# sashashura/h2o-3

Hardware: AMD Instinct MI355X
Metric: gbm_trees_per_sec (higher is better)
Workload: dtype fp32; 1 GPU; model=GBM binomial 100Mx100 ntrees=500 max_depth=8, rows=100000000, cols=100, max_depth=8, histogram_type=QuantilesGlobal, nbins=255, global_batch=100000000, parallelism=dp1

## Files before the change

h2o3_amd/models/tree/devtree.py:

```python
from __future__ import annotations

import os

import numpy as np
import torch

from ...ops import _native, tree_ops
from ...ops._native import check as _ck, ptr as _ptr, stream as _stream
from ...parallel import cloud
from ...parallel import collectives as coll
from ...utils import graphs
from .engine import _TreeBuf
from .record import FEAT, GAIN, OPT, T, rec_cols

RS = 16
_RC = rec_cols(2)
L0, L1, R0, R1, T0, T1, OK, NL, NAW = _RC.L, _RC.L + 1, _RC.R, _RC.R + 1, _RC.TOT, _RC.TOT + 1, _RC.OK, _RC.NL, _RC.NAW
ST, CT, VAL = range(_RC.width, RS)
MAX_DEPTH = 11


def _libs():
    return tree_ops._lib(), _native.get_lib("tree_split")

# ... 113 lines not shown
        self.fbase = torch.zeros(self.cap_p, dtype=i32, device=dev)
        self.lwork = torch.zeros(self.cap_l * 4, dtype=i32, device=dev)
        self.counts = torch.zeros(2, dtype=i32, device=dev)
        self.cnt = torch.zeros(self.cap_p, dtype=i32, device=dev)
        self.loff = torch.zeros(self.cap_p, dtype=i32, device=dev)
        self.roff = torch.zeros(self.cap_p, dtype=i32, device=dev)
        self.flags = torch.zeros(N // 64 + self.cap_p + 1, dtype=torch.int64, device=dev)
        self.part = self.plan_r.part(cap_h, dev)
        self.split_out = torch.zeros(n_lvl_max * max(self.Fl, 1) * 4, dtype=f64, device=dev)
        self.mask = torch.zeros(n_lvl_max * Bs, dtype=torch.uint8, device=dev)
        self.feat_i = torch.zeros(n_lvl_max, dtype=i32, device=dev)
        self.okm = torch.ones((n_lvl_max, max(self.Fl, 1)), dtype=torch.uint8, device=dev)
        if self.f0 + self.Fl > self.F:
            self.okm[:, max(0, self.F - self.f0):] = 0
        self._okm_col = None
        self.mono = torch.zeros(max(self.Fl, 1), dtype=torch.float32, device=dev)
        if bd.codes_col is not None:
            self.pcodes, self.prs, self.pfs = bd.codes_col, 1, bd.nrows_local
        else:
            self.pcodes, self.prs, self.pfs = bd.codes, bd.Fp, 1
        self.cutmat = g._cut_matrix()
        self.sampled = not drv._unit_weights
        self.wbuf = torch.ones(N, dtype=torch.float32, device=dev) if self.sampled else None
        self.colsamp = gp.col_sample_rate < 1.0 or gp.col_sample_rate_change_per_level != 1.0
        if self.colsamp:
            self.cs_elig = torch.zeros(max(self.F, 1), dtype=torch.int64, device=dev)
            self.cs_m = torch.zeros(1, dtype=torch.int32, device=dev)
            self.cs_k = torch.zeros(max(D, 1), dtype=torch.int32, device=dev)
            self.cs_seed = torch.zeros(max(D, 1), dtype=torch.int64, device=dev)
        self.gather = os.environ.get("H2O3_LEAF_GATHER", "1") != "0" and N > 0
        self.last_level = self.gather and os.environ.get("H2O3_DEV_LAST_LEVEL", "1") != "0"
        self.lg = LeafGather(self.lh, N, D, dev) if self.gather else None
        self.slot_wb = torch.zeros(n_lvl_max, dtype=i32, device=dev)
        self.graph = None
        self._hv = [None, None]
        self._k = 0

    def _scales(self):
        self.sc_r = self.plan_r.scales(self.vmax)
        self.sc_c = self.plan_c.scales(self.vmax)

    def set_tree_cols(self, mask):
        key = None if mask is None else mask.tobytes()
        if key == self._okm_col:
            return
        self._okm_col = key
        m = np.ones(self.Fpad, dtype=np.uint8)
        if mask is not None:
            m[:self.F] = np.asarray(mask, dtype=np.uint8)
        m[self.F:] = 0
        row = self._upload([m[self.f0:self.f0 + self.Fl].copy()])[0]
        self.okm.copy_(row.view(1, -1).expand_as(self.okm))

    def _upload(self, arrays):
        offs, n = [], 0
        for a in arrays:
            offs.append(n)
            n += (a.nbytes + 7) & ~7
        n = max(n, 8)
        if getattr(self, "_stg", None) is None or self._stg[0].numel() < n:
            self._stg = [torch.empty(n, dtype=torch.uint8, pin_memory=True) for _ in range(2)]
            self._stg_ev = [None, None]
            self._dstg = torch.empty(n, dtype=torch.uint8, device=self.dev)
            self._stg_i = 0
        i = self._stg_i
        self._stg_i ^= 1
# ... 68 lines not shown
        gains = g[:, :, :8].contiguous().view(torch.float64).view(W, n)
        best = torch.argmax(gains, 0)
        win = g[best, torch.arange(n, device=buf.device)]
        pk = win[:, :rb].contiguous().view(torch.float64).view(n, 13)
        rows[:, :13].copy_(pk)
        self.mask[:n * Bs].view(n, Bs).copy_(win[:, rb:])
        okf = pk[:, OK] > 0
        self.feat_i[:n].copy_(torch.where(okf, pk[:, FEAT], torch.zeros_like(pk[:, FEAT])).to(torch.int32))

    def _level(self, d, cur):
        lh, ls, gp = self.lh, self.ls, self.gp
        n = 1 << d
        Bs = self.Bs
        H, wyy = self._hist(d, cur)
        recl = self._rec_lvl(d)
        s = _stream()
        if self.colsamp:
            rp = self._rec_lvl(d - 1) if d > 0 else None
            _ck(lh.h2o_dt_colmask(d, _ptr(rp), _ptr(self.cs_elig), _ptr(self.cs_m), _ptr(self.cs_k),
                                  _ptr(self.cs_seed), self.f0, self.Fl, _ptr(self.okm), s), "dt_colmask")
        _ck(ls.h2o_split_find_b(_ptr(H), self.Fl, n, Bs, _ptr(wyy), _ptr(self.okm), _ptr(self.mono),
                                float(gp.min_rows), float(gp.min_split_improvement), float(gp.reg_lambda),
                                float(gp.reg_alpha), float(gp.gamma), 0, _ptr(self.split_out), None, 0, s),
            "split_find")
        _ck(ls.h2o_split_select2(_ptr(self.split_out), _ptr(H), self.Fl, n, Bs, self.f0, 2.0 * float(gp.min_rows), RS,
                                 _ptr(recl), _ptr(self.mask), _ptr(self.feat_i), s), "split_select2")
        if self.W > 1:
            self._merge(recl, n)
        s = _stream()
        skip = self.last_level and d == self.D - 1
        _ck(lh.h2o_dt_items2(0, _ptr(recl), n, self.D, 0, self.chunk_p, self.cap_p, _ptr(self.pwork),
                             _ptr(self.fbase), _ptr(self.slot_wb) if skip else None, _ptr(self.counts), s),
            "dt_items(part)")
        _ck(lh.h2o_part_flags(_ptr(self.pcodes), 1, self.prs, self.pfs, _ptr(self._ridx(d, cur)),
                              _ptr(self.pwork), _ptr(self.fbase), self.cap_p, _ptr(self.feat_i), _ptr(self.mask),
                              Bs, _ptr(self.flags), _ptr(self.cnt), _ptr(self.counts), s), "part_flags")
        _ck(lh.h2o_dt_offsets(_ptr(self.cnt), _ptr(self.pwork), _ptr(self.counts), _ptr(recl), n,
                              _ptr(self._rec_lvl(d + 1)), _ptr(self.loff), _ptr(self.roff), s), "dt_offsets")
        if skip:
            _ck(lh.h2o_leaf_flag_sums_dev(_ptr(self.pos[cur]), _ptr(self.pwork), _ptr(self.fbase), self.cap_p,
                                          _ptr(self.flags), _ptr(recl), self.D, 1 if self.bern else 0,
                                          _ptr(self.sums), _ptr(self.counts), s), "leaf_flag_sums_dev")
            return cur
        nxt = cur ^ 1
        if d == 0 and self.root_ident:
            _ck(lh.h2o_dt_root_leaf_iota(_ptr(recl), _ptr(self.ridx[0]), self.N, s), "dt_root_leaf_iota")
        _ck(lh.h2o_part_compact(_ptr(self._ridx(d, cur)), _ptr(self.pwork), _ptr(self.fbase), self.cap_p,
                                _ptr(self.flags), _ptr(self.loff), _ptr(self.roff), _ptr(self.ridx[nxt]),
                                _ptr(self.pos[cur]), _ptr(self.pos[nxt]), _ptr(self.counts), s),
            "part_compact")
        return nxt

    def _sequence(self):
        lh, drv = self.lh, self.drv
        s = _stream()
        y = drv.yb if self.bern else torch.nan_to_num(drv.yf)
        if not hasattr(self, "_y"):
            self._y = y.contiguous().to(torch.float32)
        f = drv._f[:, 0]
        _ck(lh.h2o_gbm_grad(_ptr(self._y), _ptr(f), _ptr(self.wbuf) if self.sampled else None,
                            1 if self.bern else 0, self.N, _ptr(self.pos[0]), _ptr(self.dbuf), s), "gbm_grad")
        if not self.root_ident:
            _ck(lh.h2o_iota_i32(_ptr(self.ridx[0]), self.N, s), "iota")
        self.rec.zero_()
        self.sums.zero_()
        _ck(lh.h2o_dt_root(_ptr(self.rec), self.N, _stream()), "dt_root")
        cur = 0
        for d in range(self.D):
            cur = self._level(d, cur)
# ... 126 lines not shown
```

h2o3_amd/ops/_abi.py:

```python
import ctypes

_TABLE = {
    "dl": """
        h2o_dl_seed_advance  i  PP
        h2o_dl_fwd           i  PPPiiifQPifP
        h2o_dl_bwd           i  PPPPPiiifQPP
        h2o_dl_update        i  PPPPPPPPPiifffffffiiiffP
        h2o_dl_softmax       i  PPPPPPPiifiP
        h2o_dl_mlp_step      i  iPPPPPPPPPPPPPPPiPPPPiifQPiP
        h2o_dl_gemm_ws       q  iii
        h2o_dl_gemm          i  iiiPqqPqqPPqP
    """,
    "dl_shap": """
        h2o_dl_shap_chunk  i
        h2o_dl_shap_lds    q  iP
        h2o_dl_shap_pairs  i  iPPPPPPPPPPiiPPqqqiiP
    """,
    "fairness": """
        h2o_fairness_lds_groups  i
        h2o_group_sketch         i  PiPPqiiidiPPPiP
    """,
    "frame": """
        h2o_rollup_multi    i  PiqiPiPP
        h2o_expand_numeric  i  PiqPPPPiiiP
# ... 6 lines not shown
        h2o_glm_wide_split_grid  i  i
        h2o_glm_wide_split       i  PiiiqPfPPPiiffPPiPPP
        h2o_glm_wide_gram        i  PiiqPiiPiP
        h2o_glm_wide_gram256     i  PiiqPiiPiiP
        h2o_gram_f64             i  PiiqPPiiqPP
        h2o_xv_f64               i  PiiqPdPP
        h2o_xtr_f64              i  PiiqPiqPP
    """,
    "kmeans": """
        h2o_kmeans_assign_resident_per_cu  i  ii
        h2o_kmeans_assign                  i  PqiPPiPPiP
        h2o_xv_resident_per_cu             i  ii
        h2o_xv                             i  PqiPiPiP
        h2o_kmeans_max_k                   i  ii
        h2o_kmeans_part_stride             q  ii
        h2o_kmeans_set_debug               v  i
        h2o_kmeans_resident_per_cu         i  iiif
        h2o_kmeans_lloyd                   i  PPqiPPiPPPPiifP
        h2o_kmeans_sums_resident_per_cu    i  ii
        h2o_kmeans_sums                    i  PPqiiPPPPifP
        h2o_kmeans_reduce                  i  PiqPP
    """,
    "metrics": """
        h2o_logit_hist    i  PPPqiPPP
        h2o_group_reduce  i  PPqiiiPP
    """,
    "tree_hist": """
        h2o_hist_quad           i  PiPPPPiiiiffPiiiPiqiiPPP
        h2o_hist_bm_set_debug   v  i
        h2o_hist_bm             i  PiPPPPiiiiffPiiPiqiiiPPPP
        h2o_iota_i32            i  PqP
        h2o_hist_build          i  PiiPPPPiiiiffPiiiPiPP
        h2o_hist_build_pk       i  PiiPPPPiiiifqPiiPiPP
        h2o_part_flags          i  PiqqPPPiPPiPPPP
        h2o_hist_sibling        i  PPPiiiiiiiPPPPPP
        h2o_child_work          i  PPPiiiiiiiiPPPP
        h2o_part_offsets        i  PPiiPPPPiiP
        h2o_part_compact        i  PPPiPPPPPPPP
        h2o_part_count          i  PiqqPPiPPiPP
        h2o_part_scatter        i  PiqqPPiPPiPPPPPPPP
        h2o_fill_nid            i  PPiPP
        h2o_leaf_pass           i  PPPPiiPPP
        h2o_seg_sum2            i  PPPPiPP
        h2o_leaf_pos            i  PPiiPPP
        h2o_col_sample          i  iiPiQPP
        h2o_leaf_scatter        i  PPiPPP
        h2o_leaf_update         i  PPiPPP
        h2o_pair_hist4          i  PiqPPPPiPiiiffPPPP
        h2o_pair_hist           i  PiqPPPPiPiiiffPPP
        h2o_gbm_grad            i  PPPiqPPP
        h2o_part_items          i  PiiiPPPP
        h2o_dt_items2           i  iPiiiiiPPPPP
        h2o_dt_items            i  iPiiiiiPPPP
        h2o_dt_offsets          i  PPPPiPPPP
        h2o_dt_sibling          i  PPPiiiiiiPPPPP
        h2o_dt_leaf_vals        i  PPiiPdPP
        h2o_dt_root             i  PqP
        h2o_dt_root_leaf_iota   i  PPqP
        h2o_leaf_scatter_dev    i  PPiPPPP
        h2o_leaf_flag_sums_dev  i  PPPiPPiiPPP
        h2o_leaf_gather_lds     i  ii
        h2o_leaf_gather_items   i  qi
        h2o_leaf_gather_dev     i  PiiiPPPPqiiPPPPPP
        h2o_dt_colmask          i  iPPPPPiiPP
    """,
    "tree_pd": """
        h2o_pd_block_threads  i  ii
# ... 48 lines not shown
```

h2o3_amd/ops/csrc/tree_hist.hip:

```cpp
#include "common.h"
#include <stdlib.h>
#include <algorithm>

template <int MODE> struct Chan { static constexpr int C = MODE == 2 ? 1 : 2; };

template <typename CodeT, int MODE, bool HAS_VB, bool POSV, bool PACK = false>
__global__ __launch_bounds__(512) void hist_build_kernel(
    const CodeT* __restrict__ codes, int Fp, const int* __restrict__ ridx,
    const float* __restrict__ va, const float* __restrict__ vb,
    const int4* __restrict__ work, int F, int Bs, int FGL, float s0, float s1,
    double* __restrict__ hist, int n_slots, double* __restrict__ wyy_out, const uint8_t* __restrict__ need,
    long long bq = 0) {
  constexpr int C = Chan<MODE>::C;
  constexpr int CL = PACK ? 1 : C;
  const int RPW = 64 / FGL;
  extern __shared__ __attribute__((aligned(16))) unsigned long long ldsq[];
  const int4 wk = work[blockIdx.x];
  if (need != nullptr && need[(size_t)wk.x * gridDim.y + blockIdx.y] == 0) return;
  const int fg0 = blockIdx.y * FGL;
  const int nf = min(FGL, F - fg0);
  const int stride_f = Bs * CL;
  const int total = FGL * stride_f;
  for (int i = threadIdx.x; i < total; i += blockDim.x) ldsq[i] = 0ull;
  __syncthreads();
// ... 823 lines not shown
    int wpre = 0, tot = 0;
#pragma unroll
    for (int w = 0; w < 4; ++w) {
      const int s = wsum[w];
      wpre += (w < wv) ? s : 0;
      tot += s;
    }
    const int lpre = wpre + incl - nl;
    const int tile_first = base;
    const int pos_before = max(0, min(p0, end) - tile_first);
    int li = lbase + lpre;
    int ri = rbase + (pos_before - lpre);
    if (p0 < end) {
#pragma unroll
      for (int k = 0; k < 16; ++k) {
        if (p0 + k < end) {
          const int dst = ((bits >> k) & 1u) ? li++ : ri++;
          out[dst] = r[k];
          if (pa) { pa_out[dst] = pa[p0 + k]; pb_out[dst] = pb[p0 + k]; }
        }
      }
    }
    const int tile_n = min(256 * 16, end - base);
    lbase += tot;
    rbase += tile_n - tot;
    __syncthreads();
  }
}
template <typename CodeT>
__global__ __launch_bounds__(256) void part_flags_kernel(
    const CodeT* __restrict__ codes, long long rs, long long fs, const int* __restrict__ ridx,
    const int4* __restrict__ work, const int* __restrict__ fbase, const int* __restrict__ feat,
    const uint8_t* __restrict__ masks, int Bs, unsigned long long* __restrict__ flags, int* __restrict__ cnt,
    const int* __restrict__ nw_dev) {
  __shared__ uint8_t m[4096];
  __shared__ int red[4];
  if (nw_dev != nullptr && (int)blockIdx.x >= nw_dev[1]) return;
  const int4 wk = work[blockIdx.x];
  const int f = feat[wk.x];
  for (int i = threadIdx.x; i < Bs; i += blockDim.x) m[i] = masks[(size_t)wk.x * Bs + i];
  __syncthreads();
  const int lane = threadIdx.x & 63, wv = threadIdx.x >> 6;
  const int end = wk.y + wk.z;
  const int fb = fbase[blockIdx.x];
  int local = 0;
  constexpr int U = 8;
  for (int base = wk.y; base < end; base += 256 * U) {
    int r[U], c[U];
#pragma unroll
    for (int u = 0; u < U; ++u) {
      const int pc = min(base + u * 256 + (int)threadIdx.x, end - 1);
      r[u] = ridx != nullptr ? ridx[pc] : pc;
    }
#pragma unroll
    for (int u = 0; u < U; ++u) c[u] = (int)codes[(size_t)r[u] * rs + (size_t)f * fs];
#pragma unroll
    for (int u = 0; u < U; ++u) {
      const int p = base + u * 256 + (int)threadIdx.x;
      const bool L = p < end && m[c[u]];
      const unsigned long long bal = __ballot(L);
      const int w0 = base + u * 256 + wv * 64;
      if (lane == 0 && w0 < end) flags[fb + (w0 - wk.y) / 64] = bal;
      local += L ? 1 : 0;
    }
  }
  local = (int)wave_sum((float)local);
  if (lane == 0) red[wv] = local;
  __syncthreads();
  if (threadIdx.x == 0) cnt[blockIdx.x] = red[0] + red[1] + red[2] + red[3];
}
// ... 235 lines not shown
}

extern "C" {

int h2o_iota_i32(int* out, long long n, hipStream_t s) {
  if (n <= 0) return 0;
  if (((uintptr_t)out & 15) != 0) return -1;
  const long long blocks = std::min<long long>((n / 4 + 255) / 256 + 1, 4096);
  hipLaunchKernelGGL(iota_i32_kernel, dim3((unsigned)blocks), dim3(256), 0, s, out, n);
  return (int)hipGetLastError();
}

int h2o_hist_build(const void* codes, int code_bytes, int Fp, const int* ridx, const float* va,
                   const float* vb, const int* work, int n_work, int F, int FG, int Bs, float s0, float s1,
                   double* hist, int n_slots, int mode, int threads, double* wyy, int posv, const uint8_t* need,
                   hipStream_t s) {
  if (n_work <= 0) return 0;
  if (code_bytes == 1)
    return launch_hist<uint8_t>(codes, Fp, ridx, va, vb, (const int4*)work, n_work, F, FG, Bs, s0, s1, hist, n_slots, mode, threads, wyy, posv, need, s);
  return launch_hist<uint16_t>(codes, Fp, ridx, va, vb, (const int4*)work, n_work, F, FG, Bs, s0, s1, hist, n_slots, mode, threads, wyy, posv, need, s);
}

int h2o_hist_build_pk(const void* codes, int code_bytes, int Fp, const int* ridx, const float* va,
                      const float* vb, const int* work, int n_work, int F, int FG, int Bs, float s1, long long bq,
                      double* hist, int n_slots, int threads, double* wyy, int posv, const uint8_t* need,
                      hipStream_t s) {
  if (n_work <= 0) return 0;
  if (bq < 0) return (int)hipErrorInvalidValue;
  if (code_bytes == 1)
    return launch_hist<uint8_t>(codes, Fp, ridx, va, vb, (const int4*)work, n_work, F, FG, Bs, 1.f, s1, hist, n_slots,
                                0, threads, wyy, posv, need, s, bq);
  return launch_hist<uint16_t>(codes, Fp, ridx, va, vb, (const int4*)work, n_work, F, FG, Bs, 1.f, s1, hist, n_slots,
                               0, threads, wyy, posv, need, s, bq);
}

int h2o_part_flags(const void* codes, int code_bytes, long long rs, long long fs, const int* ridx,
                   const int* work, const int* fbase, int n_work, const int* feat, const uint8_t* masks, int Bs,
                   unsigned long long* flags, int* cnt, const int* counts, hipStream_t s) {
  if (n_work <= 0) return 0;
  if (code_bytes == 1)
    hipLaunchKernelGGL(part_flags_kernel<uint8_t>, dim3(n_work), dim3(256), 0, s, (const uint8_t*)codes, rs, fs,
                       ridx, (const int4*)work, fbase, feat, masks, Bs, flags, cnt, counts);
  else
    hipLaunchKernelGGL(part_flags_kernel<uint16_t>, dim3(n_work), dim3(256), 0, s, (const uint16_t*)codes, rs, fs,
                       ridx, (const int4*)work, fbase, feat, masks, Bs, flags, cnt, counts);
  return (int)hipGetLastError();
}

int h2o_hist_sibling(const double* Hb, const double* Hp, const int* slots, int nb, int np, int nf, int F, int BsC,
                     int C, int clamp_mask, double* H, const double* wyy_b, const double* wyy_p, double* wyy_out,
                     const int* counts, hipStream_t s) {
  if (nb <= 0 || F <= 0) return 0;
  hipLaunchKernelGGL(hist_sibling_kernel, dim3(nb, F), dim3(256), 0, s, Hb, Hp, slots, nb, np, nf, BsC, C, clamp_mask,
                     H, wyy_b, wyy_p, wyy_out, counts);
  return (int)hipGetLastError();
}

__global__ __launch_bounds__(1024) void child_work_kernel(const long long* __restrict__ st,
                                                          const long long* __restrict__ ct,
                                                          const double* __restrict__ rec, int stride, int ok_col,
                                                          int nl_col, int wl_col, int wr_col, int n, int chunk,
                                                          int cap, int4* __restrict__ work, int* __restrict__ slots,
                                                          int* __restrict__ counts) {
  __shared__ long long wtot[2][16];
  __shared__ long long carry[2];
  const int lane = threadIdx.x & 63, wv = threadIdx.x >> 6, nwv = blockDim.x >> 6;
  if (threadIdx.x == 0) carry[0] = carry[1] = 0;
  __syncthreads();
  for (int base = 0; base < n; base += blockDim.x) {
    const int i = base + threadIdx.x;
    long long sp = 0, nch = 0, start = 0, cnt = 0;
    bool bl = true;
    if (i < n && rec[(size_t)i * stride + ok_col] > 0) {
      const long long nl = (long long)rec[(size_t)i * stride + nl_col];
      bl = rec[(size_t)i * stride + wl_col] <= rec[(size_t)i * stride + wr_col];
      cnt = bl ? nl : ct[i] - nl;
      start = bl ? st[i] : st[i] + nl;
      sp = 1;
      nch = (cnt + chunk - 1) / chunk;
// ... 926 lines not shown
      }
      sl[u] = a;
      p[u] = lo[a] + (j - pre[a]);
    }
#pragma unroll
    for (int u = 0; u < U; ++u) r[u] = ridx[p[u]];
#pragma unroll
    for (int u = 0; u < U; ++u) {
      const int4 sg = segs[sl[u]];
      int h = sg.x;
      if (sg.w >= 0) {
        const int q = p[u] - sg.y;
        h = 2 * h + (((flags[sg.w + (q >> 6)] >> (q & 63)) & 1ull) ? 1 : 2);
      }
      const long long li = (long long)r[u] - row0;
      if (j0 + u * nt < total && li >= 0 && li < nrows) v[li] = __float_as_uint(vals[h]);
    }
  }
  __syncthreads();
  float* dr = d + row0;
  for (int i = threadIdx.x * 4; i < nrows; i += nt * 4) {
    const uint4 q = *reinterpret_cast<const uint4*>(v + i);
    if (i + 3 < nrows && q.x != LG_NONE && q.y != LG_NONE && q.z != LG_NONE && q.w != LG_NONE) {
      *reinterpret_cast<uint4*>(dr + i) = q;
    } else {
      const unsigned int e[4] = {q.x, q.y, q.z, q.w};
#pragma unroll
      for (int k = 0; k < 4; ++k)
        if (i + k < nrows && e[k] != LG_NONE) dr[i + k] = __uint_as_float(e[k]);
    }
  }
}

extern "C" {

int h2o_dt_items2(int kind, const double* rec, int n, int D, int wch, int chunk, int cap, int* work, int* fbase,
                  int* slot_wb, int* counts, hipStream_t s) {
  if (n <= 0 || n > DT_MAXN || chunk <= 0 || (fbase != nullptr && chunk % 64 != 0)) return -1;
  hipLaunchKernelGGL(dt_items_kernel, dim3(1), dim3(1024), 0, s, kind, rec, n, D, wch, chunk, cap, (int4*)work, fbase,
                     slot_wb, counts);
  return (int)hipGetLastError();
}

int h2o_dt_items(int kind, const double* rec, int n, int D, int wch, int chunk, int cap, int* work, int* fbase,
                 int* counts, hipStream_t s) {
  return h2o_dt_items2(kind, rec, n, D, wch, chunk, cap, work, fbase, nullptr, counts, s);
}

int h2o_dt_offsets(const int* cnt, const int* work, const int* counts, double* rec, int n, double* rec_next, int* loff,
                   int* roff, hipStream_t s) {
  if (n <= 0 || n > DT_MAXN) return -1;
  hipLaunchKernelGGL(dt_offsets_kernel, dim3(1), dim3(1024), 0, s, cnt, (const int4*)work, counts, rec, n, rec_next,
                     loff, roff);
  return (int)hipGetLastError();
}

int h2o_dt_sibling(const double* Hb, const double* Hp, const double* rec_par, int np, int F, int BsC, int C,
                   int clamp_mask, int wch, double* H, const double* wyy_b, const double* wyy_p, double* wyy_out,
                   hipStream_t s) {
  if (np <= 0 || F <= 0) return 0;
  hipLaunchKernelGGL(dt_sibling_kernel, dim3(np, F), dim3(256), 0, s, Hb, Hp, rec_par, np, BsC, C, clamp_mask, wch, H,
                     wyy_b, wyy_p, wyy_out);
  return (int)hipGetLastError();
}

int h2o_dt_leaf_vals(double* rec, const double* sums, int nh, int D, const float* lr, double maxabs, float* vals,
                     hipStream_t s) {
// ... 135 lines not shown
```

h2o3_amd/ops/tree_ops.py:

```python
from __future__ import annotations

import math
import os
from typing import NamedTuple

import numpy as np
import torch

from . import _native
from ._native import check as _check, ptr as _ptr, stream as _stream

_LDS_BUDGET = 80 * 1024


_upload_seq = 0
_synced_upto = 0


def upload_mark():
    return _upload_seq


def host_synced(mark=None):
    global _synced_upto
# ... 517 lines not shown
    lib = _lib()
    yc, fc = y.contiguous().to(torch.float32), f.contiguous().to(torch.float32)
    wc = w.contiguous().to(torch.float32) if w is not None else None
    _check(lib.h2o_gbm_grad(_ptr(yc), _ptr(fc), _ptr(wc), mode, n, _ptr(z), _ptr(d), _stream()), "h2o_gbm_grad")
    return z


def partition(bd, ridx, ridx_out, feats, masks, starts, counts, use_native=None, chunk=16384, payload=None):
    dev = ridx.device
    n = len(starts)
    if n == 0:
        return []
    native = dev.type == "cuda" if use_native is None else use_native
    if native:
        lib = _lib()
        items = make_work(starts, counts, range(n), chunk)
        if len(items) == 0:
            return [0] * n
        work = _h2d(items, dev)
        nw = len(items)
        feat_t = _h2d(np.asarray(feats, dtype=np.int32), dev)
        masks = masks.to(torch.uint8).contiguous()
        cnt = torch.empty(nw, dtype=torch.int32, device=dev)
        if bd.codes_col is not None:
            codes, rs, fs = bd.codes_col, 1, bd.nrows_local
        else:
            codes, rs, fs = bd.codes, bd.Fp, 1
        ballot = env("H2O3_PART", "ballot") == "ballot" and (payload is None or payload[1] is None)
        if ballot:
            words = (items[:, 2].astype(np.int64) + 63) // 64
            fb_h = (np.cumsum(words) - words).astype(np.int32)
            fbase = _h2d(fb_h, dev)
            flags = torch.empty(int(words.sum()) + 1, dtype=torch.int64, device=dev)
            rc = lib.h2o_part_flags(_ptr(codes), bd.code_bytes, rs, fs, _ptr(ridx), _ptr(work), _ptr(fbase), nw,
                                    _ptr(feat_t), _ptr(masks), bd.Bs, _ptr(flags), _ptr(cnt), None, _stream())
        else:
            rc = lib.h2o_part_count(_ptr(codes), bd.code_bytes, rs, fs, _ptr(ridx), _ptr(work), nw, _ptr(feat_t),
                                    _ptr(masks), bd.Bs, _ptr(cnt), _stream())
        _check(rc, "h2o_part_count")
        cnt_h = cnt.cpu().numpy().astype(np.int64)
        slot = items[:, 0].astype(np.int64)
        nleft = np.bincount(slot, weights=cnt_h, minlength=n).astype(np.int64)
        csum = np.cumsum(cnt_h) - cnt_h
        first = np.ones(len(items), dtype=bool)
        first[1:] = slot[1:] != slot[:-1]
        first_idx = np.maximum.accumulate(np.where(first, np.arange(len(items)), 0))
        lpre = csum - csum[first_idx]
        st_arr = np.asarray(starts, dtype=np.int64)[slot]
        rpre = (items[:, 1].astype(np.int64) - st_arr) - lpre
        loff = (st_arr + lpre).astype(np.int32)
        roff = (st_arr + nleft[slot] + rpre).astype(np.int32)
        loff_d = _h2d(loff, dev)
        roff_d = _h2d(roff, dev)
        pa, pb, pa_o, pb_o = payload if payload is not None else (None, None, None, None)
        if ballot:
            _check(lib.h2o_part_compact(_ptr(ridx), _ptr(work), _ptr(fbase), nw, _ptr(flags), _ptr(loff_d),
                                        _ptr(roff_d), _ptr(ridx_out), _ptr(pa), _ptr(pa_o), None, _stream()),
                   "h2o_part_compact")
            return nleft.tolist()
        _check(lib.h2o_part_scatter(_ptr(codes), bd.code_bytes, rs, fs, _ptr(ridx), _ptr(work), nw, _ptr(feat_t),
                                    _ptr(masks), bd.Bs, _ptr(loff_d), _ptr(roff_d), _ptr(ridx_out), _ptr(pa), _ptr(pb),
                                    _ptr(pa_o), _ptr(pb_o), _stream()), "h2o_part_scatter")
        return nleft.tolist()
    out = []
    for i, (st, ct) in enumerate(zip(starts, counts)):
        seg = ridx[st: st + ct]
        if bd.codes_col is not None:
            c = bd.codes_col[feats[i]][seg.long()].to(torch.int64)
        else:
            c = bd.codes[seg.long(), feats[i]].to(torch.int64)
        left = masks[i].to(torch.bool)[c]
        l = seg[left]
        r = seg[~left]
        ridx_out[st: st + l.numel()] = l
        ridx_out[st + l.numel(): st + ct] = r
        if payload is not None:
            pa, pb, pa_o, pb_o = payload
            for src, dst in ((pa, pa_o), (pb, pb_o)):
                v = src[st: st + ct]
                dst[st: st + l.numel()] = v[left]
                dst[st + l.numel(): st + ct] = v[~left]
        out.append(int(l.numel()))
    return out


def _part_chunk(total):
    ev = env("H2O3_PART_CHUNK")
    if ev:
        return int(ev)
    return int(max(4096, min(16384, -(-int(total) // 2048 // 64) * 64)))


def iota_i32(out) -> bool:
    lib = _lib()
    if lib is None or out.dtype != torch.int32 or not out.is_cuda or out.data_ptr() % 16:
        return False
    return lib.h2o_iota_i32(_ptr(out), out.numel(), _stream()) == 0


def partition_async(bd, ridx, ridx_out, feat_d, masks, starts, counts, chunk=None, payload=None, pk=None,
                    pk_col=0):
    dev = ridx.device
    n = len(starts)
    lib = _lib()
    if chunk is None:
        chunk = _part_chunk(sum(counts))
    nleft = torch.empty(n, dtype=torch.int64, device=dev)
    st = np.asarray(starts, dtype=np.int64).reshape(-1)
    ct = np.asarray(counts, dtype=np.int64).reshape(-1)
    nch = (ct + chunk - 1) // chunk
    nw = int(nch.sum())
    if nw == 0:
        nleft.zero_()
        if pk is not None:
            pk[:, pk_col] = 0.0
        return nleft
    wd = (ct + 63) // 64
    total_words = int(wd.sum())
    buf = torch.empty(13 * nw, dtype=torch.int32, device=dev)
    meta = buf[: 8 * nw].view(torch.int64)
    work = buf[8 * nw: 12 * nw]
    fbase = buf[12 * nw:]
    if chunk % 64 == 0 and env("H2O3_PART_ITEMS", "dev") == "dev":
        seg = _h2d(np.concatenate([st, ct, np.cumsum(nch) - nch, np.cumsum(wd) - wd]), dev)
        _check(lib.h2o_part_items(_ptr(seg), n, chunk, nw, _ptr(work), _ptr(meta), _ptr(fbase), _stream()),
               "h2o_part_items")
    else:
        items = make_work(starts, counts, range(n), chunk)
        words = (items[:, 2].astype(np.int64) + 63) // 64
        fb_h = (np.cumsum(words) - words).astype(np.int64)
        slot = items[:, 0].astype(np.int64)
        first = np.ones(nw, dtype=bool)
        first[1:] = slot[1:] != slot[:-1]
        first_idx = np.maximum.accumulate(np.where(first, np.arange(nw), 0))
        st_arr = st[slot]
        pos = items[:, 1].astype(np.int64) - st_arr
        buf.copy_(_h2d(np.concatenate([np.stack([slot, first_idx, st_arr, pos], 0).reshape(-1).view(np.int32),
                                       items.reshape(-1), fb_h.astype(np.int32)]), dev))
    feat_t = feat_d if feat_d.dtype == torch.int32 else feat_d.to(torch.int32)
    masks = masks if masks.dtype == torch.uint8 else masks.to(torch.uint8)
    cnt = torch.empty(nw, dtype=torch.int32, device=dev)
    if bd.codes_col is not None:
        codes, rs, fs = bd.codes_col, 1, bd.nrows_local
    else:
        codes, rs, fs = bd.codes, bd.Fp, 1
    flags = torch.empty(total_words + 1, dtype=torch.int64, device=dev)
    _check(lib.h2o_part_flags(_ptr(codes), bd.code_bytes, rs, fs, _ptr(ridx), _ptr(work), _ptr(fbase), nw,
                              _ptr(feat_t), _ptr(masks), bd.Bs, _ptr(flags), _ptr(cnt), None, _stream()),
           "h2o_part_flags")
    loff = torch.empty(nw, dtype=torch.int32, device=dev)
    roff = torch.empty(nw, dtype=torch.int32, device=dev)
    stride = pk.stride(0) if pk is not None else 0
    _check(lib.h2o_part_offsets(_ptr(cnt), _ptr(meta), nw, n, _ptr(loff), _ptr(roff), _ptr(nleft), _ptr(pk),
                                stride, pk_col, _stream()), "h2o_part_offsets")
    pa, _, pa_o, _ = payload if payload is not None else (None, None, None, None)
    _check(lib.h2o_part_compact(_ptr(ridx), _ptr(work), _ptr(fbase), nw, _ptr(flags), _ptr(loff), _ptr(roff),
                                _ptr(ridx_out), _ptr(pa), _ptr(pa_o), None, _stream()), "h2o_part_compact")
    return nleft


def hist_build_dev(bd, ridx, va, vb, mode, rec, rec_cols, starts, counts, vmax, posv=False, unit_w=False,
                   target_blocks=None):
    dev = ridx.device
    if dev.type != "cuda":
        return None
    total = int(sum(counts))
    plan = hist_plan(bd, mode, unit_w, (total + 1) // 2, target_blocks)
    if plan.kernel not in ("bm", "quad"):
        return None
    lib = _lib()
    n = len(starts)
    C = channels(mode)
    chunk = plan.chunk
    cap = n + total // chunk + 1
    stc = np.concatenate([np.asarray(starts, dtype=np.int64), np.asarray(counts, dtype=np.int64)])
    stc_d = _h2d(stc, dev)
    ibuf = torch.empty(4 * cap + 3 * n + 2, dtype=torch.int32, device=dev)
    work, slots, cnts = ibuf[:4 * cap], ibuf[4 * cap:4 * cap + 3 * n], ibuf[4 * cap + 3 * n:]
    ok_c, nl_c, wl_c, wr_c = rec_cols
    _check(lib.h2o_child_work(_ptr(stc_d), _ptr(stc_d[n:]), _ptr(rec), rec.stride(0), ok_c, nl_c, wl_c, wr_c, n, chunk,
                              cap, _ptr(work), _ptr(slots), _ptr(cnts), _stream()), "h2o_child_work")
# ... 166 lines not shown
```

Before: 69.94 trees/s.

## Add slab-based partition flag kernel that streams feature columns through LDS windows

Adds a row-slab partition-flags path for deep levels (depth >= 5, up to 1024 nodes) with column-major 1-byte codes. Each block loads a 64K-row window of one split feature's codes into LDS and classifies the rows that fall in that window. This replaces scattered random gathers from huge feature columns with coalesced streaming reads. A device-side rule decides whether to use the slab path, based on distinct features versus rows, and falls back to the original kernel otherwise. The cost is extra small kernels (rule, zero, binary-search bounds), atomics on flags and counts, and high LDS use.

```diff
diff --git a/h2o3_amd/models/tree/devtree.py b/h2o3_amd/models/tree/devtree.py
--- a/h2o3_amd/models/tree/devtree.py
+++ b/h2o3_amd/models/tree/devtree.py
@@ -169,6 +169,7 @@
         self.last_level = self.gather and os.environ.get("H2O3_DEV_LAST_LEVEL", "1") != "0"
         self.lg = LeafGather(self.lh, N, D, dev) if self.gather else None
         self.slot_wb = torch.zeros(n_lvl_max, dtype=i32, device=dev)
+        self.slab = tree_ops.PartSlab(N, n_lvl_max, dev) if bd.codes_col is not None and N > 0 else None
         self.graph = None
         self._hv = [None, None]
         self._k = 0
@@ -303,9 +304,10 @@
         _ck(lh.h2o_dt_items2(0, _ptr(recl), n, self.D, 0, self.chunk_p, self.cap_p, _ptr(self.pwork),
                              _ptr(self.fbase), _ptr(self.slot_wb) if skip else None, _ptr(self.counts), s),
             "dt_items(part)")
-        _ck(lh.h2o_part_flags(_ptr(self.pcodes), 1, self.prs, self.pfs, _ptr(self._ridx(d, cur)),
-                              _ptr(self.pwork), _ptr(self.fbase), self.cap_p, _ptr(self.feat_i), _ptr(self.mask),
-                              Bs, _ptr(self.flags), _ptr(self.cnt), _ptr(self.counts), s), "part_flags")
+        slab = self.slab if self.slab is not None and self.slab.eligible(d) else None
+        _ck(tree_ops.part_flags(lh, self.pcodes, 1, self.prs, self.pfs, self._ridx(d, cur), self.pwork, self.fbase,
+                                self.cap_p, self.feat_i, self.mask, Bs, self.flags, self.cnt, self.counts, slab,
+                                recl, n, self.chunk_p), "part_flags")
         _ck(lh.h2o_dt_offsets(_ptr(self.cnt), _ptr(self.pwork), _ptr(self.counts), _ptr(recl), n,
                               _ptr(self._rec_lvl(d + 1)), _ptr(self.loff), _ptr(self.roff), s), "dt_offsets")
         if skip:
diff --git a/h2o3_amd/ops/_abi.py b/h2o3_amd/ops/_abi.py
--- a/h2o3_amd/ops/_abi.py
+++ b/h2o3_amd/ops/_abi.py
@@ -62,7 +62,7 @@
         h2o_iota_i32            i  PqP
         h2o_hist_build          i  PiiPPPPiiiiffPiiiPiPP
         h2o_hist_build_pk       i  PiiPPPPiiiifqPiiPiPP
-        h2o_part_flags          i  PiqqPPPiPPiPPPP
+        h2o_part_flags          i  PiqqPPPiPPiPPPPiqiiidPPqP
         h2o_hist_sibling        i  PPPiiiiiiiPPPPPP
         h2o_child_work          i  PPPiiiiiiiiPPPP
         h2o_part_offsets        i  PPiiPPPPiiP
diff --git a/h2o3_amd/ops/csrc/tree_hist.hip b/h2o3_amd/ops/csrc/tree_hist.hip
--- a/h2o3_amd/ops/csrc/tree_hist.hip
+++ b/h2o3_amd/ops/csrc/tree_hist.hip
@@ -879,10 +879,11 @@
     const CodeT* __restrict__ codes, long long rs, long long fs, const int* __restrict__ ridx,
     const int4* __restrict__ work, const int* __restrict__ fbase, const int* __restrict__ feat,
     const uint8_t* __restrict__ masks, int Bs, unsigned long long* __restrict__ flags, int* __restrict__ cnt,
-    const int* __restrict__ nw_dev) {
+    const int* __restrict__ nw_dev, const int* __restrict__ slab) {
   __shared__ uint8_t m[4096];
   __shared__ int red[4];
   if (nw_dev != nullptr && (int)blockIdx.x >= nw_dev[1]) return;
+  if (slab != nullptr && slab[1] != 0) return;
   const int4 wk = work[blockIdx.x];
   const int f = feat[wk.x];
   for (int i = threadIdx.x; i < Bs; i += blockDim.x) m[i] = masks[(size_t)wk.x * Bs + i];
@@ -1184,19 +1185,6 @@
                                 0, threads, wyy, posv, need, s, bq);
   return launch_hist<uint16_t>(codes, Fp, ridx, va, vb, (const int4*)work, n_work, F, FG, Bs, 1.f, s1, hist, n_slots,
                                0, threads, wyy, posv, need, s, bq);
-}
-
-int h2o_part_flags(const void* codes, int code_bytes, long long rs, long long fs, const int* ridx,
-                   const int* work, const int* fbase, int n_work, const int* feat, const uint8_t* masks, int Bs,
-                   unsigned long long* flags, int* cnt, const int* counts, hipStream_t s) {
-  if (n_work <= 0) return 0;
-  if (code_bytes == 1)
-    hipLaunchKernelGGL(part_flags_kernel<uint8_t>, dim3(n_work), dim3(256), 0, s, (const uint8_t*)codes, rs, fs,
-                       ridx, (const int4*)work, fbase, feat, masks, Bs, flags, cnt, counts);
-  else
-    hipLaunchKernelGGL(part_flags_kernel<uint16_t>, dim3(n_work), dim3(256), 0, s, (const uint16_t*)codes, rs, fs,
-                       ridx, (const int4*)work, fbase, feat, masks, Bs, flags, cnt, counts);
-  return (int)hipGetLastError();
 }
 
 int h2o_hist_sibling(const double* Hb, const double* Hp, const int* slots, int nb, int np, int nf, int F, int BsC,
@@ -2189,7 +2177,278 @@
   }
 }
 
+#define PS_MAXN 1024
+#define PS_NT 1024
+
+__global__ __launch_bounds__(PS_NT) void ps_rule_kernel(const double* __restrict__ rec, int n,
+                                                        const int* __restrict__ feat, long long N, int chunk,
+                                                        int rule, double slab_c, int* __restrict__ slab) {
+  __shared__ int sfeat[PS_MAXN];
+  __shared__ long long wtot[3][16];
+  __shared__ int ktot[16];
+  const int i = threadIdx.x, lane = i & 63, wv = i >> 6;
+  constexpr int nwv = PS_NT / 64;
+  const long long ct = i < n ? max((long long)rec[(size_t)i * DT_RS + DT_CT], 0ll) : 0;
+  const long long nch = (ct + chunk - 1) / chunk, nwd = (ct + 63) / 64;
+  sfeat[i] = (i < n && ct > 0) ? feat[i] : -1;
+  long long a = nch, b = nwd, r = ct;
+#pragma unroll
+  for (int o = 1; o < 64; o <<= 1) {
+    const long long ta = __shfl_up(a, o, 64), tb = __shfl_up(b, o, 64), tr = __shfl_up(r, o, 64);
+    if (lane >= o) { a += ta; b += tb; r += tr; }
+  }
+  if (lane == 63) { wtot[0][wv] = a; wtot[1][wv] = b; wtot[2][wv] = r; }
+  __syncthreads();
+  bool first = sfeat[i] >= 0;
+  for (int j = 0; j < i && first; ++j) first = sfeat[j] != sfeat[i];
+  const int kw = __popcll(__ballot(first));
+  if (lane == 0) ktot[wv] = kw;
+  long long oa = 0, ob = 0, rows = 0;
+  for (int w = 0; w < nwv; ++w) {
+    oa += (w < wv) ? wtot[0][w] : 0;
+    ob += (w < wv) ? wtot[1][w] : 0;
+    rows += wtot[2][w];
+  }
+  if (i < n) {
+    slab[2 + i] = (int)(ob + b - nwd);
+    slab[2 + n + i] = (int)(oa + a - nch);
+  }
+  __syncthreads();
+  if (i == 0) {
+    int k = 0;
+    for (int w = 0; w < nwv; ++w) k += ktot[w];
+    slab[0] = k;
+    slab[1] = (k > 0 && (rule == 1 || (rule == 2 && (double)k * (double)N <= slab_c * (double)rows))) ? 1 : 0;
+  }
+}
+
+__global__ __launch_bounds__(256) void ps_zero_kernel(const int* __restrict__ slab, const int* __restrict__ counts,
+                                                      unsigned long long* __restrict__ flags, long long nwords,
+                                                      int* __restrict__ cnt, int cap) {
+  if (slab[1] == 0) return;
+  const long long stride = (long long)gridDim.x * blockDim.x;
+  const long long t = (long long)blockIdx.x * blockDim.x + threadIdx.x;
+  for (long long i = t; i < nwords; i += stride) flags[i] = 0ull;
+  const int ni = min(counts[1], cap);
+  for (long long i = t; i < ni; i += stride) cnt[i] = 0;
+}
+
+__global__ __launch_bounds__(256) void ps_bounds_kernel(const int* __restrict__ ridx, const double* __restrict__ rec,
+                                                        int n, long long N, int R, int nb,
+                                                        const int* __restrict__ slab, int* __restrict__ T) {
+  if (slab[1] == 0) return;
+  const long long e = (long long)blockIdx.x * blockDim.x + threadIdx.x;
+  if (e >= (long long)(nb + 1) * n) return;
+  const int b = (int)(e / n), s = (int)(e % n);
+  const double* r = rec + (size_t)s * DT_RS;
+  const long long st = min(max((long long)r[DT_ST], 0ll), N);
+  const long long ct = min(max((long long)r[DT_CT], 0ll), N - st);
+  const long long key = (long long)b * R;
+  int lo = (int)st, hi = (int)(st + ct);
+  while (lo < hi) {
+    const int mid = lo + ((hi - lo) >> 1);
+    if ((long long)ridx[mid] < key) lo = mid + 1; else hi = mid;
+  }
+  T[e] = lo;
+}
+
+__global__ __launch_bounds__(PS_NT) __attribute__((amdgpu_waves_per_eu(8))) void ps_flags_kernel(
+    const uint8_t* __restrict__ codes, long long fs, const int* __restrict__ ridx, const int* __restrict__ T, int n,
+    const int* __restrict__ feat, const uint8_t* __restrict__ masks, int Bs, int chunk, int cap, long long N, int R,
+    const int* __restrict__ slab, unsigned long long* __restrict__ flags, long long nwords, int* __restrict__ cnt) {
+  extern __shared__ __attribute__((aligned(16))) unsigned char ps_lds[];
+  if (slab[1] == 0) return;
+  uint8_t* win = ps_lds;
+  unsigned int* mb = reinterpret_cast<unsigned int*>(ps_lds + R + 16);
+  int* sa = reinterpret_cast<int*>(mb + (size_t)n * 8);
+  int* se = sa + n;
+  int* sst = se + n;
+  int* sen = sst + n;
+  int* sf = sen + n;
+  int* swb = sf + n;
+  int* sib = swb + n;
+  int* pre = sib + n;
+  __shared__ int wred[16];
+  constexpr int NONE = 0x7fffffff;
+  const int tid = threadIdx.x, lane = tid & 63, wv = tid >> 6;
+  constexpr int nwv = PS_NT / 64;
+  const int b = blockIdx.x, nb = gridDim.x;
+  const long long row0 = (long long)b * R;
+  const int nrows = (int)min((long long)R, N - row0);
+  if (tid < n) {
+    const int a = T[(size_t)b * n + tid], e = T[(size_t)(b + 1) * n + tid];
+    sa[tid] = a;
+    se[tid] = e;
+    sst[tid] = T[tid];
+    sen[tid] = T[(size_t)nb * n + tid];
+    sf[tid] = e > a ? feat[tid] : NONE;
+    swb[tid] = slab[2 + tid];
+    sib[tid] = slab[2 + n + tid];
+  }
+  for (int i = tid; i < n * 8; i += PS_NT) {
+    const int s = i >> 3, w = i & 7;
+    unsigned int bits = 0;
+    for (int k = 0; k < 32; ++k) {
+      const int bin = w * 32 + k;
+      if (bin < Bs && masks[(size_t)s * Bs + bin]) bits |= 1u << k;
+    }
+    mb[i] = bits;
+  }
+  __syncthreads();
+  int last = -1;
+  for (;;) {
+    int m = NONE;
+    if (tid < n) {
+      const int v = sf[tid];
+      if (v > last) m = v;
+    }
+#pragma unroll
+    for (int o = 32; o > 0; o >>= 1) m = min(m, __shfl_xor(m, o, 64));
+    if (lane == 0) wred[wv] = m;
+    __syncthreads();
+    m = NONE;
+#pragma unroll
+    for (int w = 0; w < nwv; ++w) m = min(m, wred[w]);
+    if (m == NONE) break;
+    const int f = m;
+    last = f;
+    const uint8_t* src = codes + (size_t)f * fs + row0;
+    const int mis = (int)(reinterpret_cast<uintptr_t>(src) & 15);
+    const uint8_t* src0 = src - mis;
+    for (int c = tid * 16; c < mis + nrows; c += PS_NT * 16) {
+      if (c >= mis && c + 16 <= mis + nrows) {
+        *reinterpret_cast<uint4*>(win + c) = *reinterpret_cast<const uint4*>(src0 + c);
+      } else {
+        for (int k = 0; k < 16; ++k) {
+          const int o = c + k;
+          if (o >= mis && o < mis + nrows) win[o] = src0[o];
+        }
+      }
+    }
+    int nw = 0;
+    if (tid < n && sf[tid] == f) nw = ((se[tid] - 1 - sst[tid]) >> 6) - ((sa[tid] - sst[tid]) >> 6) + 1;
+    int x = nw;
+#pragma unroll
+    for (int o = 1; o < 64; o <<= 1) {
+      const int t = __shfl_up(x, o, 64);
+      if (lane >= o) x += t;
+    }
+    __syncthreads();
+    if (lane == 63) wred[wv] = x;
+    __syncthreads();
+    int off = 0, total = 0;
+#pragma unroll
+    for (int w = 0; w < nwv; ++w) { off += (w < wv) ? wred[w] : 0; total += wred[w]; }
+    if (tid < n) pre[tid] = off + x - nw;
+    if (tid == 0) pre[n] = total;
+    __syncthreads();
+    const int j0 = (int)((long long)total * wv / nwv), j1 = (int)((long long)total * (wv + 1) / nwv);
+    for (int jb = j0; jb < j1; jb += 64) {
+      const int nbw = min(64, j1 - jb);
+      int w_sl = 0, w_p0 = 0, w_lo = 0, w_hi = 0, w_item = -1;
+      long long w_word = -1;
+      bool w_whole = false;
+      if (lane < nbw) {
+        const int jj = jb + lane;
+        int lo = 0, hi = n - 1;
+        while (lo < hi) {
+          const int mid = (lo + hi + 1) >> 1;
+          if (pre[mid] <= jj) lo = mid; else hi = mid - 1;
+        }
+        const int a = sa[lo], e = se[lo], st = sst[lo];
+        const int ww = ((a - st) >> 6) + (jj - pre[lo]);
+        w_sl = lo;
+        w_p0 = st + ww * 64;
+        w_lo = max(a, w_p0);
+        w_hi = min(e, w_p0 + 64);
+        w_whole = w_p0 >= a && min(w_p0 + 64, sen[lo]) <= e;
+        w_word = (long long)swb[lo] + ww;
+        w_item = sib[lo] + (int)((unsigned)(ww * 64) / (unsigned)chunk);
+      }
+      unsigned long long mybal = 0ull;
+      constexpr int U = 8;
+      for (int t0 = 0; t0 < nbw; t0 += U) {
+        int r[U];
+        bool vd[U];
+#pragma unroll
+        for (int u = 0; u < U; ++u) {
+          const int t = min(t0 + u, nbw - 1);
+          const int p = __builtin_amdgcn_readlane(w_p0, t) + lane;
+          vd[u] = t0 + u < nbw && p >= __builtin_amdgcn_readlane(w_lo, t) && p < __builtin_amdgcn_readlane(w_hi, t);
+          r[u] = vd[u] ? ridx[p] : 0;
+        }
+#pragma unroll
+        for (int u = 0; u < U; ++u) {
+          const int t = min(t0 + u, nbw - 1);
+          const int sl = __builtin_amdgcn_readlane(w_sl, t);
+          const int li = min(max((int)((long long)r[u] - row0), 0), nrows - 1);
+          const int c = win[mis + li];
+          const bool L = vd[u] && ((mb[sl * 8 + (c >> 5)] >> (c & 31)) & 1u);
+          const unsigned long long bal = __ballot(L);
+          if (lane == t0 + u) mybal = bal;
+        }
+      }
+      if (lane < nbw && w_word >= 0 && w_word < nwords) {
+        if (w_whole) flags[w_word] = mybal;
+        else if (mybal != 0ull) atomicOr(&flags[w_word], mybal);
+      }
+      int x = __popcll(mybal);
+      const int own = x;
+#pragma unroll
+      for (int o = 1; o < 64; o <<= 1) {
+        const int t = __shfl_up(x, o, 64);
+        if (lane >= o) x += t;
+      }
+      const int prev = __shfl_up(w_item, 1, 64);
+      const bool head = lane < nbw && (lane == 0 || prev != w_item);
+      const unsigned long long heads = __ballot(head);
+      const unsigned long long above = lane == 63 ? 0ull : (heads >> (lane + 1)) << (lane + 1);
+      const int rend = (above != 0ull ? __ffsll((long long)above) - 1 : nbw) - 1;
+      const int sum = __shfl(x, rend, 64) - (x - own);
+      if (head && sum != 0 && w_item >= 0 && w_item < cap) atomicAdd(&cnt[w_item], sum);
+    }
+    __syncthreads();
+  }
+}
+
 extern "C" {
+
+int h2o_part_flags(const void* codes, int code_bytes, long long rs, long long fs, const int* ridx,
+                   const int* work, const int* fbase, int n_work, const int* feat, const uint8_t* masks, int Bs,
+                   unsigned long long* flags, int* cnt, const int* counts, const double* rec_lvl, int n, long long N,
+                   int R, int chunk, int rule, double slab_c, int* slab, int* T, long long nwords, hipStream_t s) {
+  if (n_work <= 0) return 0;
+  if (slab != nullptr && N > 0) {
+    if (code_bytes != 1 || rs != 1 || ridx == nullptr || counts == nullptr || rec_lvl == nullptr || T == nullptr ||
+        n <= 0 || n > PS_MAXN || R < 256 || R % 16 != 0 || Bs <= 0 || Bs > 256 || chunk <= 0 || chunk % 64 != 0 ||
+        nwords <= 0 || N > (1ll << 31) - (1 << 24))
+      return -1;
+    const int lds = R + 16 + n * 32 + (8 * n + 1) * (int)sizeof(int);
+    if (lds > 160 * 1024 - 256) return -1;
+    static int lds_set = 0;
+    if (lds > lds_set) {
+      if (hipFuncSetAttribute((const void*)ps_flags_kernel, hipFuncAttributeMaxDynamicSharedMemorySize, lds) !=
+          hipSuccess)
+        return -2;
+      lds_set = lds;
+    }
+    const int nb = (int)((N + R - 1) / R);
+    const long long ne = (long long)(nb + 1) * n;
+    hipLaunchKernelGGL(ps_rule_kernel, dim3(1), dim3(PS_NT), 0, s, rec_lvl, n, feat, N, chunk, rule, slab_c, slab);
+    hipLaunchKernelGGL(ps_zero_kernel, dim3(1024), dim3(256), 0, s, slab, counts, flags, nwords, cnt, n_work);
+    hipLaunchKernelGGL(ps_bounds_kernel, dim3((unsigned)((ne + 255) / 256)), dim3(256), 0, s, ridx, rec_lvl, n, N,
+                       R, nb, slab, T);
+    hipLaunchKernelGGL(ps_flags_kernel, dim3(nb), dim3(PS_NT), lds, s, (const uint8_t*)codes, fs, ridx, T, n, feat,
+                       masks, Bs, chunk, n_work, N, R, slab, flags, nwords, cnt);
+  }
+  if (code_bytes == 1)
+    hipLaunchKernelGGL(part_flags_kernel<uint8_t>, dim3(n_work), dim3(256), 0, s, (const uint8_t*)codes, rs, fs,
+                       ridx, (const int4*)work, fbase, feat, masks, Bs, flags, cnt, counts, slab);
+  else
+    hipLaunchKernelGGL(part_flags_kernel<uint16_t>, dim3(n_work), dim3(256), 0, s, (const uint16_t*)codes, rs, fs,
+                       ridx, (const int4*)work, fbase, feat, masks, Bs, flags, cnt, counts, slab);
+  return (int)hipGetLastError();
+}
 
 int h2o_dt_items2(int kind, const double* rec, int n, int D, int wch, int chunk, int cap, int* work, int* fbase,
                   int* slot_wb, int* counts, hipStream_t s) {
diff --git a/h2o3_amd/ops/tree_ops.py b/h2o3_amd/ops/tree_ops.py
--- a/h2o3_amd/ops/tree_ops.py
+++ b/h2o3_amd/ops/tree_ops.py
@@ -573,8 +573,8 @@
             fb_h = (np.cumsum(words) - words).astype(np.int32)
             fbase = _h2d(fb_h, dev)
             flags = torch.empty(int(words.sum()) + 1, dtype=torch.int64, device=dev)
-            rc = lib.h2o_part_flags(_ptr(codes), bd.code_bytes, rs, fs, _ptr(ridx), _ptr(work), _ptr(fbase), nw,
-                                    _ptr(feat_t), _ptr(masks), bd.Bs, _ptr(flags), _ptr(cnt), None, _stream())
+            rc = part_flags(lib, codes, bd.code_bytes, rs, fs, ridx, work, fbase, nw, feat_t, masks, bd.Bs, flags, cnt,
+                            None)
         else:
             rc = lib.h2o_part_count(_ptr(codes), bd.code_bytes, rs, fs, _ptr(ridx), _ptr(work), nw, _ptr(feat_t),
                                     _ptr(masks), bd.Bs, _ptr(cnt), _stream())
@@ -632,6 +632,51 @@
     return int(max(4096, min(16384, -(-int(total) // 2048 // 64) * 64)))
 
 
+PART_SLAB_R = 65536
+PART_SLAB_MIN_LEVEL = 5
+PART_SLAB_C = 16.0
+PART_SLAB_MIN_ROWS = 50_000_000
+PART_SLAB_MAXN = 1024
+
+
+class PartSlab:
+
+    def __init__(self, N, n_max, dev, mode=None, min_level=None, R=None, c=None):
+        mode = env("H2O3_PART_SLAB", "auto") if mode is None else str(mode)
+        if mode not in ("auto", "0", "1"):
+            raise ValueError(f"H2O3_PART_SLAB={mode!r}: auto, 0 or 1")
+        self.N = int(N)
+        self.rule = {"0": 0, "1": 1, "auto": 2}[mode]
+        self.min_level = max(1, int(env("H2O3_PART_SLAB_MIN", PART_SLAB_MIN_LEVEL) if min_level is None
+                                    else min_level))
+        self.R = int(env("H2O3_PART_SLAB_R", PART_SLAB_R) if R is None else R)
+        self.c = float(PART_SLAB_C if c is None else c)
+        self.n_max = min(int(n_max), PART_SLAB_MAXN)
+        if self.R < 256 or self.R % 16 or self.R + 16 + 64 * self.n_max + 4 > 160 * 1024 - 256:
+            raise ValueError(f"H2O3_PART_SLAB_R={self.R}: a multiple of 16, >= 256, window + slot tables within LDS")
+        nb = -(-self.N // self.R)
+        self.T = torch.zeros((nb + 1) * self.n_max, dtype=torch.int32, device=dev)
+        self.word = torch.zeros(2 + 2 * self.n_max, dtype=torch.int32, device=dev)
+
+    def eligible(self, d):
+        if self.rule == 0 or d < self.min_level or (1 << d) > self.n_max:
+            return False
+        return self.N >= PART_SLAB_MIN_ROWS if self.rule == 2 else self.N > 0
+
+
+def part_flags(lib, codes, code_bytes, rs, fs, ridx, work, fbase, n_work, feat, masks, Bs, flags, cnt, counts,
+               slab=None, rec_lvl=None, n=0, chunk=0):
+    if slab is None:
+        return lib.h2o_part_flags(_ptr(codes), code_bytes, rs, fs, _ptr(ridx), _ptr(work), _ptr(fbase), n_work,
+                                  _ptr(feat), _ptr(masks), Bs, _ptr(flags), _ptr(cnt), _ptr(counts), None, 0, 0, 0,
+                                  0, 0, 0.0, None, None, 0, _stream())
+    nwords = min(flags.numel(), slab.N // 64 + n + 1)
+    return lib.h2o_part_flags(_ptr(codes), code_bytes, rs, fs, _ptr(ridx), _ptr(work), _ptr(fbase), n_work,
+                              _ptr(feat), _ptr(masks), Bs, _ptr(flags), _ptr(cnt), _ptr(counts), _ptr(rec_lvl), n,
+                              slab.N, slab.R, chunk, slab.rule, slab.c, _ptr(slab.word), _ptr(slab.T), nwords,
+                              _stream())
+
+
 def iota_i32(out) -> bool:
     lib = _lib()
     if lib is None or out.dtype != torch.int32 or not out.is_cuda or out.data_ptr() % 16:
@@ -686,8 +731,7 @@
     else:
         codes, rs, fs = bd.codes, bd.Fp, 1
     flags = torch.empty(total_words + 1, dtype=torch.int64, device=dev)
-    _check(lib.h2o_part_flags(_ptr(codes), bd.code_bytes, rs, fs, _ptr(ridx), _ptr(work), _ptr(fbase), nw,
-                              _ptr(feat_t), _ptr(masks), bd.Bs, _ptr(flags), _ptr(cnt), None, _stream()),
+    _check(part_flags(lib, codes, bd.code_bytes, rs, fs, ridx, work, fbase, nw, feat_t, masks, bd.Bs, flags, cnt, None),
            "h2o_part_flags")
     loff = torch.empty(nw, dtype=torch.int32, device=dev)
     roff = torch.empty(nw, dtype=torch.int32, device=dev)
```

Result: no change. 70.22 trees/s (median of 6 runs) (+0.4%).
